# LuoGroup2023/PanTax

Hardware: AMD Instinct MI355X
Metric: PAO wall-time (s) + Mreads/s: packed reads + DB (graphs and their unique-trio index) resident in HBM -> abundance tables; the metric's own GAF -> abundance quantity is value_gaf_to_tables (files -> tables, never `value`) (higher is better)
Workload: dtype int64+f64

## Files before the change

### pantax_amd/csrc/common.hpp

```cpp
#pragma once
#include <hip/hip_runtime.h>
#include <cstdint>
#include <cstdio>
#include <map>
#include <functional>
#include <mutex>
#include <cstring>
#include <atomic>
#include <string>
#include <vector>
#include "../../include/pantax_hip.h"

#ifndef TRIO_LH_PACK
#define TRIO_LH_PACK 0
#endif
namespace ptx {

struct Ctx;
#if TRIO_LH_PACK
using trio_len_t = uint2;
#else
using trio_len_t = uint32_t;
#endif

// ... 36 lines not shown
    void release() {
        if (p && owned) dev_cache_free(p, cap, dev);
        p = nullptr;
        n = 0;
        cap = 0;
        owned = true;
    }
    void view(void *ptr, size_t count) {
        release();
        p = static_cast<T *>(ptr);
        n = count;
        owned = false;
    }
    hipError_t alloc(size_t count) {
        if (count <= n && p) return hipSuccess;
        release();
        hipError_t e = dev_cache_alloc((void **)&p, (count ? count : 1) * sizeof(T), &cap, &dev);
        if (e == hipSuccess) n = count ? count : 1;
        return e;
    }
    size_t bytes() const { return n * sizeof(T); }
    void take(DevBuf &o) { release(); p = o.p; n = o.n; cap = o.cap; dev = o.dev; owned = o.owned; o.p = nullptr; o.n = 0; o.cap = 0; o.owned = true; }
};

struct PinBuf {
    uint8_t *p = nullptr;
    size_t n = 0;
    PinBuf() = default;
    PinBuf(const PinBuf &) = delete;
    PinBuf &operator=(const PinBuf &) = delete;
    ~PinBuf() { release(); }
    void release() { if (p) (void)hipHostFree(p); p = nullptr; n = 0; }
    hipError_t reserve(size_t bytes) {
        if (bytes <= n && p) return hipSuccess;
        release();
        size_t want = bytes < 65536 ? 65536 : bytes;
        hipError_t e = hipHostMalloc((void **)&p, want, hipHostMallocDefault);
        if (e == hipSuccess) n = want;
        return e;
    }
};

struct TimedLaunch {
    const char *name;
    hipEvent_t start, stop;
};

struct CtxConfig {
    bool trace = false;
    int stage_threads = 32;
    int stage_ch_mb = 0;
    bool stream_prio = true;
    int dev_cache_gb = -1;
    bool numa_bind = true;
    uint64_t gaf_piece_bytes = 0;
    int db_groups = 0;
    uint64_t db_path_steps_max = 0;
    std::string trio_path;
    std::string trio_rows;
    int uniq_hash = -1;
    std::string mask;
    std::string row_sort;
    std::string objective;
    std::string read_strain_route, evidence_route, depth_route, near_miss_route, hap_pairs_route, fit_route, bootstrap_route, dropout_route;
    uint64_t bootstrap_rows_max = 0;
    uint64_t dropout_patterns_max = 0;
    bool dropout_yardstick = false;
    int hap_pairs_chunk = 0;
    int depth_grid = 0;
    int near_miss_words = 0;
    bool cov_general = false;
    std::string cov_long;
    int covl_shape = -1;
    bool cov_count = false;
    int cov_clean_async = -1;
    bool cov_self_clean = false;
    bool walk_sum_in_bin = false;
    int ncs_prefix_min = 48;
    bool ncs_no_prefix = false;
    bool cov_arena_verify = false;
    int cov_item_groups = 0;
    int tv_u = 4, tv_rounds = 4, tf_u = 8, tf_rounds = 1, rows_u = 1, tb_slots = 256, trio_xcd = 3, cov_shape = -1, covf_shape = -1, cov_xcd = 0, group_bucket_bits = 0;
    uint32_t tv_ablate = 0, cov_ablate = 0, ssn_ablate = 0;
    bool trio_two_pass = false;
    std::string bin_route;
    std::string node_pass;
    std::string node_bits;
    int node_bits_words = 0;
    std::string lad_shape;
    std::string scan_tile;
    std::string ssn_keys;
    bool ssn_poison_keys = false;
    int ssn_ties_async = -1;
    bool no_absent_skip = false;
    bool ssn_debug = false, scan_no_huge = false, flag_rank_chained = false, ratio_kernel = false, mask_pass = false, trio_free_at_filter = false,
         trio_after_step = false;
};
int ctx_set_option(CtxConfig &cfg, const char *name, const char *value);

struct NumaInfo {
    int node = -1;
    std::vector<int> cpus;
};

struct Ctx {
    std::recursive_mutex mu;
    CtxConfig cfg;
    NumaInfo numa;
    int device = 0;
    hipStream_t stream = nullptr;
    hipStream_t stream_main = nullptr;
    hipStream_t stream2 = nullptr;
    hipStream_t stream_up = nullptr;
    hipEvent_t ev_fork = nullptr;
    hipEvent_t ev_ssn_fork = nullptr, ev_ssn_join = nullptr;
    hipEvent_t ev_seq = nullptr;
    std::string err;
    std::mutex err_mu;
    bool timing = false;
    std::string timing_filter;
    std::vector<TimedLaunch> pending;
    std::vector<std::pair<hipEvent_t, hipEvent_t>> free_events;
    std::map<std::string, std::pair<uint64_t, double>> acc;
    int n_cu = 256;
    DevBuf<uint64_t> d_scalars;
    DevBuf<uint32_t> d_scan_ws;
    uint32_t scan_epoch = 0;
    DevBuf<uint32_t> d_scan_ws2;
    uint32_t scan_epoch2 = 0;
    PinBuf pin_down;
    PinBuf pin_text;
    PinBuf pin_up;
    size_t pin_up_off = 0;
    hipEvent_t pin_up_ev[2][2] = {{nullptr, nullptr}, {nullptr, nullptr}};
    bool pin_up_ev_set[2] = {false, false};
};

struct KTimer {
    Ctx *ctx;
    hipEvent_t start = nullptr, stop = nullptr;
    const char *name;
    KTimer(Ctx *c, const char *nm);
    ~KTimer();
};

int collect_timings(Ctx *ctx);

constexpr uint32_t BIN_PREFIX = 2048;
size_t bin_counter_words(uint32_t S);
size_t bin_result_words(uint32_t S);
struct Db; struct Reads;
int species_profile_launch(Ctx *ctx, const Db *db, const Reads *rd, const unsigned long long *d_counters, const double *d_avg_len, int filtered,
                           uint8_t *d_keep, double *d_absolute);
void species_profile_host(uint32_t S, const uint32_t *head_qlen, size_t n_head, const int64_t *read_count, const int64_t *base_sum,
                          const int64_t *less_multi, const int64_t *uniq_count, const double *avg_len, int filtered, uint8_t *keep_out,
                          double *absolute_out, double *abundance_out);
constexpr int PATH_TILE = 1024;
constexpr int LAD_MAXP = 64;
constexpr int LAD_WIDE_NW = 4;
constexpr int LAD_WIDEP = 64 * LAD_WIDE_NW;

struct LadBatch {
    uint32_t S = 0;
    bool prezeroed = false;
    std::vector<int32_t> h_p;
    std::vector<uint32_t> h_cand;
// ... 383 lines not shown
```

### pantax_amd/csrc/ctx.cpp

```cpp
#include <exception>
#include <cstdarg>
#include <algorithm>
#include <atomic>
#include <cstring>
#include <functional>
#include <chrono>
#include <condition_variable>
#include <cstdio>
#include <mutex>
#include <thread>
#include <unistd.h>
#include <fcntl.h>
#include <sched.h>
#include <pthread.h>
#include <sys/syscall.h>
#include <fstream>
#include <cctype>
#include <cstddef>
#include <cstdlib>
#include "common.hpp"
#include "lad.hpp"

namespace ptx {

static thread_local std::string g_init_err;
static thread_local std::string g_thread_err;
static thread_local const Ctx *g_thread_err_ctx = nullptr;

int fail(Ctx *ctx, int code, const char *fmt, ...) {
    char buf[1024];
    va_list ap;
    va_start(ap, fmt);
    vsnprintf(buf, sizeof(buf), fmt, ap);
    va_end(ap);
    if (ctx) {
        { std::lock_guard<std::mutex> g(ctx->err_mu); ctx->err = buf; }
        g_thread_err = buf; g_thread_err_ctx = ctx;
    } else g_init_err = buf;
    return code;
}

KTimer::KTimer(Ctx *c, const char *nm) : ctx(c), name(nm) {
    if (!ctx->timing) return;
    if (!ctx->timing_filter.empty()) {
        const std::string &f = ctx->timing_filter;
        const size_t len = std::strlen(nm);
        bool hit = false;
        for (size_t pos = 0; pos <= f.size() && !hit;) {
            const size_t bar = std::min(f.find('|', pos), f.size());
            hit = bar - pos == len && f.compare(pos, len, nm) == 0;
            pos = bar + 1;
        }
        if (!hit) return;
    }
    if (!ctx->free_events.empty()) {
        start = ctx->free_events.back().first;
        stop = ctx->free_events.back().second;
        ctx->free_events.pop_back();
    } else {
        if (hipEventCreate(&start) != hipSuccess || hipEventCreate(&stop) != hipSuccess) { start = stop = nullptr; return; }
    }
    (void)hipEventRecord(start, ctx->stream);
}
KTimer::~KTimer() {
    if (!start) return;
    (void)hipEventRecord(stop, ctx->stream);
    ctx->pending.push_back({name, start, stop});
}

int collect_timings(Ctx *ctx) {
    if (ctx->pending.empty()) return 0;
    PTX_HIP(ctx, hipStreamSynchronize(ctx->stream));
    for (auto &t : ctx->pending) {
        float ms = 0.f;
        if (hipEventElapsedTime(&ms, t.start, t.stop) == hipSuccess) {
            auto &a = ctx->acc[t.name];
            a.first += 1;
            a.second += ms;
        }
        ctx->free_events.push_back({t.start, t.stop});
    }
    ctx->pending.clear();
    return 0;
}

namespace {
enum OptKind { O_BOOL, O_INT, O_U32, O_U64, O_STR };
struct OptDesc { const char *name; OptKind kind; size_t off; };
#define OPT(nm, kind, field) {nm, kind, offsetof(CtxConfig, field)}
const OptDesc OPTIONS[] = {
    OPT("hip_trace", O_BOOL, trace), OPT("stage_threads", O_INT, stage_threads), OPT("stage_ch_mb", O_INT, stage_ch_mb), OPT("stream_prio", O_BOOL, stream_prio), OPT("numa_bind", O_BOOL, numa_bind), OPT("dev_cache_gb", O_INT, dev_cache_gb),
    OPT("gaf_piece_bytes", O_U64, gaf_piece_bytes), OPT("db_path_steps_max", O_U64, db_path_steps_max), OPT("db_groups", O_INT, db_groups), OPT("trio_path", O_STR, trio_path), OPT("trio_rows", O_STR, trio_rows), OPT("trio_two_pass", O_BOOL, trio_two_pass), OPT("uniq_hash", O_INT, uniq_hash),
    OPT("mask", O_STR, mask), OPT("row_sort", O_STR, row_sort), OPT("objective", O_STR, objective), OPT("read_strain_route", O_STR, read_strain_route), OPT("evidence_route", O_STR, evidence_route), OPT("depth_route", O_STR, depth_route), OPT("depth_grid", O_INT, depth_grid), OPT("near_miss_route", O_STR, near_miss_route), OPT("near_miss_words", O_INT, near_miss_words), OPT("hap_pairs_route", O_STR, hap_pairs_route), OPT("fit_route", O_STR, fit_route), OPT("bootstrap_route", O_STR, bootstrap_route), OPT("bootstrap_rows_max", O_U64, bootstrap_rows_max), OPT("dropout_route", O_STR, dropout_route), OPT("dropout_patterns_max", O_U64, dropout_patterns_max), OPT("dropout_yardstick", O_BOOL, dropout_yardstick), OPT("hap_pairs_chunk", O_INT, hap_pairs_chunk),
    OPT("cov_general", O_BOOL, cov_general), OPT("cov_long", O_STR, cov_long), OPT("covl_shape", O_INT, covl_shape), OPT("cov_count", O_BOOL, cov_count), OPT("cov_self_clean", O_BOOL, cov_self_clean), OPT("cov_clean_async", O_INT, cov_clean_async), OPT("cov_arena_verify", O_BOOL, cov_arena_verify), OPT("ncs_no_prefix", O_BOOL, ncs_no_prefix), OPT("ncs_prefix_min", O_INT, ncs_prefix_min), OPT("walk_sum_in_bin", O_BOOL, walk_sum_in_bin), OPT("cov_item_groups", O_INT, cov_item_groups), OPT("tv_u", O_INT, tv_u), OPT("tv_rounds", O_INT, tv_rounds), OPT("tf_u", O_INT, tf_u), OPT("tf_rounds", O_INT, tf_rounds),
    OPT("rows_u", O_INT, rows_u), OPT("tb_slots", O_INT, tb_slots), OPT("trio_xcd", O_INT, trio_xcd), OPT("cov_shape", O_INT, cov_shape),
    OPT("covf_shape", O_INT, covf_shape), OPT("cov_xcd", O_INT, cov_xcd), OPT("group_bucket_bits", O_INT, group_bucket_bits), OPT("tv_ablate", O_U32, tv_ablate),
    OPT("cov_ablate", O_U32, cov_ablate), OPT("ssn_ablate", O_U32, ssn_ablate), OPT("no_absent_skip", O_BOOL, no_absent_skip), OPT("node_pass", O_STR, node_pass), OPT("bin_route", O_STR, bin_route), OPT("node_bits", O_STR, node_bits), OPT("node_bits_words", O_INT, node_bits_words), OPT("lad_shape", O_STR, lad_shape), OPT("ssn_debug", O_BOOL, ssn_debug),
    OPT("ssn_keys", O_STR, ssn_keys), OPT("ssn_poison_keys", O_BOOL, ssn_poison_keys), OPT("ssn_ties_async", O_INT, ssn_ties_async),
    OPT("scan_no_huge", O_BOOL, scan_no_huge), OPT("scan_tile", O_STR, scan_tile), OPT("flag_rank_chained", O_BOOL, flag_rank_chained), OPT("ratio_kernel", O_BOOL, ratio_kernel),
    OPT("mask_pass", O_BOOL, mask_pass), OPT("trio_free_at_filter", O_BOOL, trio_free_at_filter), OPT("trio_after_step", O_BOOL, trio_after_step),
};
#undef OPT
}

int ctx_set_option(CtxConfig &cfg, const char *name, const char *value) {
    if (!name) return PANTAX_HIP_E_INVALID;
    static const CtxConfig defaults;
    for (const OptDesc &o : OPTIONS) {
        if (std::strcmp(o.name, name) != 0) continue;
        char *dst = reinterpret_cast<char *>(&cfg) + o.off;
        const char *def = reinterpret_cast<const char *>(&defaults) + o.off;
        char *end = nullptr;
        switch (o.kind) {
        case O_BOOL: *reinterpret_cast<bool *>(dst) = value ? !(value[0] == '0' || value[0] == '\0' || value[0] == 'n' || value[0] == 'f') : *reinterpret_cast<const bool *>(def); return 0;
        case O_INT: { if (!value) { *reinterpret_cast<int *>(dst) = *reinterpret_cast<const int *>(def); return 0; }
                      const long v = std::strtol(value, &end, 10); if (end == value) return PANTAX_HIP_E_INVALID; *reinterpret_cast<int *>(dst) = (int)v; return 0; }
        case O_U32: { if (!value) { *reinterpret_cast<uint32_t *>(dst) = *reinterpret_cast<const uint32_t *>(def); return 0; }
                      const unsigned long long v = std::strtoull(value, &end, 10); if (end == value) return PANTAX_HIP_E_INVALID; *reinterpret_cast<uint32_t *>(dst) = (uint32_t)v; return 0; }
        case O_U64: { if (!value) { *reinterpret_cast<uint64_t *>(dst) = *reinterpret_cast<const uint64_t *>(def); return 0; }
                      const unsigned long long v = std::strtoull(value, &end, 10); if (end == value) return PANTAX_HIP_E_INVALID; *reinterpret_cast<uint64_t *>(dst) = (uint64_t)v; return 0; }
        case O_STR: *reinterpret_cast<std::string *>(dst) = value ? value : ""; return 0;
        }
    }
    return PANTAX_HIP_E_INVALID;
}

static void config_from_env(CtxConfig &cfg) {
    for (const OptDesc &o : OPTIONS) {
        std::string env = "PANTAX_";
        for (const char *p = o.name; *p; ++p) env += (char)std::toupper((unsigned char)*p);
        if (const char *v = std::getenv(env.c_str())) (void)ctx_set_option(cfg, o.name, v);
    }
}

}

using namespace ptx;

extern "C" {

const char *pantax_hip_version(void) { return "pantax-hip 0.1.0 (gfx950)"; }

int pantax_hip_set_option(pantax_hip_ctx *ctx, const char *name, const char *value) {
    if (!ctx || !name) return PANTAX_HIP_E_INVALID;
    std::lock_guard<std::recursive_mutex> ptx_lock__(ctx->mu);
    const int rc = ctx_set_option(ctx->cfg, name, value);
    if (rc == 0 && std::strcmp(name, "dev_cache_gb") == 0) dev_cache_set_max(ctx->cfg.dev_cache_gb < 0 ? -1 : (long long)ctx->cfg.dev_cache_gb << 30);
    return rc == 0 ? 0 : fail(ctx, rc, "set_option: unknown option or unparsable value: %s=%s", name, value ? value : "(default)");
}

const char *pantax_hip_lad_shape_name(const pantax_hip_ctx *ctx, uint32_t n_species, int max_columns) {
    if (!ctx) return nullptr;
    return lad_shape_name(lad_shape(ctx->cfg.lad_shape, n_species, ctx->n_cu, max_columns));
}

const char *pantax_hip_last_error(const pantax_hip_ctx *ctx) {
    if (!ctx) return g_init_err.c_str();
    if (g_thread_err_ctx == ctx) return g_thread_err.c_str();
    std::lock_guard<std::mutex> g(const_cast<pantax_hip_ctx *>(ctx)->err_mu);
    g_thread_err = ctx->err;
    return g_thread_err.c_str();
}

int pantax_hip_init(pantax_hip_ctx **out, const int *device_ids, int n_devices) {
    if (!out) return PANTAX_HIP_E_INVALID;
    *out = nullptr;
    if (n_devices != 1) return fail(nullptr, PANTAX_HIP_E_INVALID, "one ctx drives one GPU (one process per GPU); n_devices=%d", n_devices);
    int count = 0;
    hipError_t e = hipGetDeviceCount(&count);
    if (e != hipSuccess || count == 0)
        return fail(nullptr, PANTAX_HIP_E_NO_DEVICE, "no HIP device visible (%s); this library has no CPU path",
                    e == hipSuccess ? "count=0" : hipGetErrorString(e));
    int dev = device_ids ? device_ids[0] : 0;
    if (dev < 0 || dev >= count) return fail(nullptr, PANTAX_HIP_E_INVALID, "device id %d out of range (count %d)", dev, count);
    hipDeviceProp_t prop;
    if ((e = hipGetDeviceProperties(&prop, dev)) != hipSuccess) return fail(nullptr, PANTAX_HIP_E_HIP, "hipGetDeviceProperties: %s", hipGetErrorString(e));
    if (strncmp(prop.gcnArchName, "gfx950", 6) != 0)
        return fail(nullptr, PANTAX_HIP_E_NO_DEVICE, "device %d is %s; this build carries gfx950 code only", dev, prop.gcnArchName);
    if ((e = hipSetDevice(dev)) != hipSuccess) return fail(nullptr, PANTAX_HIP_E_HIP, "hipSetDevice: %s", hipGetErrorString(e));
// ... 542 lines not shown
```

### pantax_amd/csrc/stage_cov.hip

```cpp
#include <chrono>
#include <cstdio>
#include <cstdlib>
#include "common.hpp"
#include "primitives.hpp"
#include "wave.hpp"
#include "cov_plan.hpp"
#include "cov_device.hpp"
#pragma clang diagnostic ignored "-Wbitwise-instead-of-logical"

namespace ptx {

template <bool WITH_TRIO, int U, int PASSES, int WIN, bool LONG = false>
__global__ void __launch_bounds__(COV_BLOCK) coverage_fast_kernel(
    const uint2 *__restrict__ items, const uint32_t *__restrict__ group_slot, const uint4 *__restrict__ read_rec, const uint2 *__restrict__ slot_rec,
    const uint32_t *__restrict__ node_id, const uint8_t *__restrict__ step_code, const uint8_t *__restrict__ active,
    const uint4 *__restrict__ node_rec, const uint64_t *__restrict__ bit_off, uint64_t V, unsigned long long *__restrict__ bases,
    uint32_t *__restrict__ bitmap, uint32_t *__restrict__ full, const uint2 *__restrict__ trio_ent, unsigned long long *__restrict__ trio_bases,
    unsigned long long *__restrict__ n_abort, uint32_t ablate, int blk_shift,
    const uint32_t *__restrict__ long_sum = nullptr, const uint32_t *__restrict__ long_len0 = nullptr, uint32_t only_long = 0u,
    uint32_t chunk_groups = 0u, uint32_t total_groups = 0u, uint32_t win_back = 0u, const uint32_t *__restrict__ item_sel = nullptr) {
    constexpr int WAVES = COV_BLOCK / 64;
    const int lane = threadIdx.x & 63, wave = threadIdx.x >> 6;
    uint32_t g0, n_groups;
    if constexpr (LONG) { g0 = blockIdx.x * chunk_groups; n_groups = min(g0 + chunk_groups, total_groups); }
    else { const uint2 item = items[item_sel ? item_sel[blockIdx.x] : blockIdx.x]; g0 = item.x; n_groups = item.y; }
    for (int i = threadIdx.x; i < (int)(cov_lds_bytes(WIN) / 4); i += COV_BLOCK) s_cov[i] = 0;
    uint32_t wlo = 0, win_n = 0, mark_n = 0, bit0_lo = 0, bwn = 0;
    uint64_t bw0 = 0;
#pragma unroll 1
    for (uint32_t g = g0; g < n_groups && win_n == 0; ++g) {
        const uint32_t gs = group_slot[g];
        if (gs == NO_SLOT) continue;
        const uint2 sr0 = slot_rec[gs];
        if ((int)sr0.x < 0 || !active[sr0.x]) continue;
        const uint32_t id0 = node_id[(uint64_t)g * 64], v0 = id0 + sr0.y, in_blk = id0 & ((1u << blk_shift) - 1u);
        const uint32_t back = LONG ? win_back : in_blk + 64u;
        wlo = (v0 > back ? v0 - back : 0u) & ~63u;
        win_n = WIN;
        const uint64_t b_lo = bit_off[wlo], b_hi = bit_off[min((uint64_t)wlo + WIN, V)];
        bw0 = b_lo >> 5;
        bit0_lo = (uint32_t)(bw0 << 5);
        bwn = COV_BWIN;
        mark_n = (b_hi - (bw0 << 5) <= (uint64_t)COV_BWIN * 32) ? (uint32_t)min((uint64_t)WIN, V - wlo) : 0u;
    }
    __builtin_amdgcn_fence(__ATOMIC_RELEASE, "workgroup", "local");
    __builtin_amdgcn_s_barrier();
    __builtin_amdgcn_fence(__ATOMIC_ACQUIRE, "workgroup", "local");
#ifndef COV_NO_PREFETCH
    uint32_t n_code[U], n_id[U], n_gs[U];
    {
        const uint32_t gw0 = g0 + (uint32_t)(wave * U);
#pragma unroll
        for (int u = 0; u < U; ++u) {
            const uint32_t g = gw0 + (uint32_t)u < n_groups ? gw0 + (uint32_t)u : (gw0 < n_groups ? gw0 : g0);
            const uint64_t t = (uint64_t)g * 64 + lane;
            n_code[u] = step_code[t]; n_id[u] = node_id[t]; n_gs[u] = group_slot[g];
        }
    }
#endif
#if !defined(COV_NO_PF2) && !defined(COV_NO_PREFETCH)
    constexpr bool PF2 = !LONG;
#else
    constexpr bool PF2 = false;
#endif
    uint32_t c_code[U], c_id[U], c_gs[U];
    uint4 c_rr[U];
    uint2 c_sr[U];
    bool c_run[U];
#pragma unroll
    for (int u = 0; u < U; ++u) c_run[u] = false;
    if constexpr (PF2) {
        const uint32_t gw0 = g0 + (uint32_t)(wave * U), gw1 = gw0 + (uint32_t)(WAVES * U);
#pragma unroll
        for (int u = 0; u < U; ++u) {
            c_code[u] = n_code[u]; c_id[u] = n_id[u]; c_gs[u] = n_gs[u];
            const uint32_t g = gw1 + (uint32_t)u < n_groups ? gw1 + (uint32_t)u : (gw0 < n_groups ? gw0 : g0);
            const uint64_t t = (uint64_t)g * 64 + lane;
            n_code[u] = step_code[t]; n_id[u] = node_id[t]; n_gs[u] = group_slot[g];
            const bool pad0 = c_code[u] == STEP_PAD;
            const bool run0 = (gw0 + (uint32_t)u < n_groups) & any1(!pad0) & none1(!pad0 & ((c_code[u] & STEP_LONG) != 0u));
            const uint32_t sl = slot_in_group(c_gs[u], c_code[u], lane);
            const uint32_t slot = (pad0 | !run0) ? (c_gs[u] == NO_SLOT ? 0u : c_gs[u]) : sl;
            c_rr[u] = read_rec[slot]; c_sr[u] = slot_rec[slot];
            c_run[u] = run0;
        }
    }
#pragma unroll 1
    for (int pass = 0;; ++pass) {
        const uint32_t gw = g0 + (uint32_t)((pass * WAVES + wave) * U);
        if (gw >= n_groups) break;
        uint32_t code[U], id[U], gs[U];
        bool run[U];
        uint4 rr[U];
        uint2 sr[U];
#ifndef COV_NO_PREFETCH
        if constexpr (PF2) {
            const uint32_t gn = gw + (uint32_t)(WAVES * U), g2 = gn + (uint32_t)(WAVES * U);
            uint32_t m_code[U], m_id[U], m_gs[U];
#pragma unroll
            for (int u = 0; u < U; ++u) {
                run[u] = c_run[u];
                code[u] = c_code[u]; id[u] = c_id[u]; gs[u] = c_gs[u]; rr[u] = c_rr[u]; sr[u] = c_sr[u];
                const uint32_t g = g2 + (uint32_t)u < n_groups ? g2 + (uint32_t)u : gw;
                const uint64_t t = (uint64_t)g * 64 + lane;
                m_code[u] = step_code[t]; m_id[u] = node_id[t]; m_gs[u] = group_slot[g];
                const bool padn = n_code[u] == STEP_PAD;
                const bool runn = (gn + (uint32_t)u < n_groups) & any1(!padn) & none1(!padn & ((n_code[u] & STEP_LONG) != 0u));
                const uint32_t sl = slot_in_group(n_gs[u], n_code[u], lane);
                const uint32_t slot = (padn | !runn) ? (n_gs[u] == NO_SLOT ? 0u : n_gs[u]) : sl;
                c_rr[u] = read_rec[slot]; c_sr[u] = slot_rec[slot];
                c_run[u] = runn;
                c_code[u] = n_code[u]; c_id[u] = n_id[u]; c_gs[u] = n_gs[u];
                n_code[u] = m_code[u]; n_id[u] = m_id[u]; n_gs[u] = m_gs[u];
            }
        } else
        {
            const uint32_t gn = gw + (uint32_t)(WAVES * U);
#pragma unroll
            for (int u = 0; u < U; ++u) {
                run[u] = gw + (uint32_t)u < n_groups;
                code[u] = n_code[u]; id[u] = n_id[u]; gs[u] = n_gs[u];
                const uint32_t g = gn + (uint32_t)u < n_groups ? gn + (uint32_t)u : gw;
                const uint64_t t = (uint64_t)g * 64 + lane;
                n_code[u] = step_code[t]; n_id[u] = node_id[t]; n_gs[u] = group_slot[g];
            }
        }
#else
#pragma unroll
        for (int u = 0; u < U; ++u) {
            const uint32_t g = gw + (uint32_t)u;
            run[u] = g < n_groups;
            const uint64_t t = (uint64_t)(run[u] ? g : gw) * 64 + lane;
            code[u] = step_code[t]; id[u] = node_id[t];
            gs[u] = group_slot[run[u] ? g : gw];
        }
#endif
        bool pad[U];
        uint32_t ll0[U], lsum[U];
#pragma unroll
        for (int u = 0; u < U; ++u) {
            pad[u] = code[u] == STEP_PAD;
            if constexpr (!PF2) {
                const bool has_long = any1(!pad[u] & ((code[u] & STEP_LONG) != 0u));
                run[u] = run[u] & any1(!pad[u]) & (LONG ? (has_long | (only_long == 0u)) : !has_long);
            }
            const uint32_t sl = slot_in_group(gs[u], code[u], lane);
            const uint32_t slot = (pad[u] | !run[u]) ? (gs[u] == NO_SLOT ? 0u : gs[u]) : sl;
            if constexpr (!PF2) { rr[u] = read_rec[slot]; sr[u] = slot_rec[slot]; }
            if constexpr (LONG) { ll0[u] = long_len0[slot]; lsum[u] = long_sum[slot]; }
        }
        uint32_t h_id1[U], h_id2[U], h_codes[U];
        if constexpr (LONG) {
#pragma unroll
            for (int u = 0; u < U; ++u) {
                const uint32_t gu = (uint32_t)__builtin_amdgcn_readfirstlane((int)(gw + (uint32_t)u));
                const uint64_t t0 = (uint64_t)(run[u] && gu != 0u ? gu : 1u) * 64;
                h_id1[u] = node_id[t0 - 1]; h_id2[u] = node_id[t0 - 2];
                h_codes[u] = *reinterpret_cast<const uint32_t *>(step_code + t0 - 4);
            }
        }
        uint4 nr[U];
        uint32_t v[U], act[U];
        bool ok[U];
#pragma unroll
        for (int u = 0; u < U; ++u) {
            ok[u] = run[u] & !pad[u] & ((int)sr[u].x >= 0);
            v[u] = ok[u] ? id[u] + sr[u].y : wlo;
            nr[u] = node_rec[v[u]];
            act[u] = active[ok[u] ? sr[u].x : 0u];
        }
        uint32_t idf[U], i0_[U], hv1[U], hv2[U];
        uint4 nrh1[U], nrh2[U];
        if constexpr (LONG) {
#pragma unroll
            for (int u = 0; u < U; ++u) {
                idf[u] = node_id[rr[u].x];
                const uint32_t gbase = (gw + (uint32_t)u) * 64u;
                const bool ok0 = __builtin_amdgcn_readfirstlane((int)ok[u]) != 0;
                i0_[u] = ok0 ? (uint32_t)__builtin_amdgcn_readfirstlane((int)(gbase - rr[u].x)) : 0u;
                const uint32_t delta0 = (uint32_t)__builtin_amdgcn_readfirstlane((int)sr[u].y);
                hv1[u] = i0_[u] >= 1u ? h_id1[u] + delta0 : wlo;
                hv2[u] = i0_[u] >= 2u ? h_id2[u] + delta0 : wlo;
                nrh1[u] = node_rec[hv1[u]]; nrh2[u] = node_rec[hv2[u]];
            }
        }
        uint32_t i_[U], nl[U], len0[U], nh[U], hx[U], tlo[U], thi[U];
        uint2 e0[U], e1[U];
        bool live[U], single[U], dead_read[U], cross[U];
        int dist[U];
#pragma unroll
        for (int u = 0; u < U; ++u) {
            const uint32_t gbase = (gw + (uint32_t)u) * 64u;
            i_[u] = gbase + (uint32_t)lane - rr[u].x;
            ok[u] = ok[u] & (act[u] != 0u);
            nl[u] = ok[u] ? nr[u].z : 0u;
            if constexpr (LONG) {
                dist[u] = (int)min(ok[u] ? i_[u] : 0u, (uint32_t)lane);
                cross[u] = ok[u] & (i_[u] > (uint32_t)lane);
                const uint32_t in_wave = __shfl(nl[u], lane - dist[u]);
                len0[u] = cross[u] ? ll0[u] : in_wave;
            } else
            len0[u] = __shfl(nl[u], lane - (int)i_[u]);
            uint32_t v2 = wave_shr1(wave_shr1(v[u]));
            uint32_t hw1 = wave_shr1(nr[u].w), hy1 = wave_shr1(nr[u].y);
            if constexpr (LONG) {
                v2 = lane == 0 ? hv2[u] : lane == 1 ? hv1[u] : v2;
                hw1 = lane == 0 ? nrh1[u].w : hw1; hy1 = lane == 0 ? nrh1[u].y : hy1;
            }
            single[u] = rr[u].y == 1u;
            dead_read[u] = !single[u] & (rr[u].z > len0[u]);
            live[u] = ok[u] & !dead_read[u] & !(single[u] & (rr[u].w < rr[u].z));
            nh[u] = 0; hx[u] = 0; tlo[u] = 0; thi[u] = 0;
            e0[u] = make_uint2(0u, 0u); e1[u] = e0[u];
            if (WITH_TRIO && !ABL(4u)) {
                hx[u] = hw1;
                tlo[u] = min(v[u], v2); thi[u] = max(v[u], v2);
                nh[u] = (live[u] & (i_[u] >= 2u) & ((nr_filter(hy1) & nr_pair_bit(tlo[u], thi[u])) != 0u)) ? nr_rows(hy1) : 0u;
                const EntPair ep = *reinterpret_cast<const EntPair *>(trio_ent + (nh[u] ? hx[u] : 0u));
                e0[u] = make_uint2(ep.a, ep.b); e1[u] = make_uint2(ep.c, ep.d);
            }
        }
#pragma unroll
        for (int u = 0; u < U; ++u) {
            const uint32_t k = rr[u].y, ps = rr[u].z, pe = rr[u].w, i = i_[u];
            if (any1(ok[u] & dead_read[u] & (i == 0u))) { if (ok[u] & dead_read[u] & (i == 0u)) atomicAdd(n_abort, 1ull); }
            const uint32_t contrib = (live[u] & !single[u]) ? (i == 0u ? nl[u] - ps : nl[u]) : 0u;
            const uint32_t pexcl = wave_incl_scan_dpp(contrib) - contrib;
            uint32_t seen = pexcl - __shfl(pexcl, lane - (LONG ? dist[u] : (int)i));
            if constexpr (LONG) seen = cross[u] ? lsum[u] - ps : seen;
            const uint32_t tgt = pe - ps;
            uint32_t aln = nl[u];
            if (i + 1u == k) aln = ((pe >= ps) & (tgt > seen)) ? tgt - seen : 0u;
            if (i == 0u) aln = single[u] ? tgt : nl[u] - ps;
            const uint32_t sidx = i == 0u ? ps : 0u;
            uint32_t hi = sidx + aln;
            if (hi > nl[u]) hi = nl[u];
            const bool markable = live[u] & (hi > sidx) & !(single[u] & !((ps < pe) & (pe <= nl[u])));
            const uint32_t dupd = code[u] & STEP_DIST;
            bool earlier = dupd != 0u, at_step0 = dupd == i;
            if constexpr (LONG) {
                const bool lc = (code[u] & STEP_LONG) != 0u;
                const uint32_t id_first = cross[u] ? idf[u] : __shfl(id[u], lane - dist[u]);
                earlier = lc ? (code[u] & 1u) != 0u : earlier;
                at_step0 = lc ? id[u] == id_first : at_step0;
            }
            const uint32_t rl = !live[u] ? 0u : !earlier ? aln : (at_step0 ? len0[u] - ps : nl[u]);
            const uint32_t off = v[u] - wlo;
            const bool inw = off < win_n;
            if (live[u] & !earlier & (aln != 0u) && !ABL(2u)) {
                if (inw & (aln < (1u << 18))) atomicAdd(&S_WIN(off), aln);
                else atomicAdd(&bases[v[u]], (unsigned long long)aln);
            }
// ... 228 lines not shown
    db->cov_arena_clean = false;
    db->cov_arena_sig = sig;
    if (rd->R && rd->T_pad && rd->n_long && rd->long_sums_db != 0 && rd->long_sums_db == db->uid) {
    } else if (rd->R && rd->T_pad && rd->n_long) {
        PTX_HIP(ctx, hipMemsetAsync(rd->d_long_sum.p, 0, rd->R * sizeof(uint32_t), ctx->stream));
        KTimer t(ctx, "walk_sum_kernel");
        const bool eager = (uint64_t)rd->n_long * 2 > rd->n_slots;
        hipLaunchKernelGGL((eager ? walk_sum_kernel<4, true> : walk_sum_kernel<4, false>), dim3(grid_for(rd->T_pad / 4 + 1, 256, ctx->n_cu * 16)), dim3(256), 0, ctx->stream, rd->T_pad, rd->d_g_group_slot.p,
                           rd->d_g_step_dup.p, rd->d_g_read_rec.p, rd->d_g_slot_rec.p, rd->d_g_node_id.p, db->d_node_len.p, rd->d_long_sum.p,
                           rd->d_long_len0.p);
    }
    PTX_HIP(ctx, hipGetLastError());
    db->cov_prepared = true;
    return 0;
}

int coverage_arena_clean_async(Ctx *ctx, Db *db) {
    if (!db->d_cov_arena.p || !db->cov_arena_total || !ctx->stream2) return 0;
    uint8_t *f_ptr = db->d_cov_arena.p;
    const size_t f_n = db->cov_arena_total;
    if (!db->ev_cov_read) PTX_HIP(ctx, hipEventCreateWithFlags(&db->ev_cov_read, hipEventDisableTiming));
    if (!db->ev_cov_clean) PTX_HIP(ctx, hipEventCreateWithFlags(&db->ev_cov_clean, hipEventDisableTiming));
    PTX_HIP(ctx, hipEventRecord(db->ev_cov_read, ctx->stream));
    PTX_HIP(ctx, hipStreamWaitEvent(ctx->stream2, db->ev_cov_read, 0));
    hipStream_t main_stream = ctx->stream;
    ctx->stream_main = main_stream; ctx->stream = ctx->stream2;
    int rc;
    rc = zero_fill(ctx, f_ptr, f_n);
    const hipError_t e = hipEventRecord(db->ev_cov_clean, ctx->stream2);
    ctx->stream = main_stream; ctx->stream_main = nullptr;
    if (rc != 0) return rc;
    PTX_HIP(ctx, e);
    db->cov_done = false;
    db->cov_arena_clean = true; db->cov_clean_pending = true;
    return 0;
}

struct CovLap {
    Ctx *ctx;
    bool on;
    std::chrono::steady_clock::time_point prev = std::chrono::steady_clock::now();
    void operator()(const char *what) {
        if (!on) return;
        (void)hipStreamSynchronize(ctx->stream);
        const auto now = std::chrono::steady_clock::now();
        std::fprintf(stderr, "[node_coverage]        %-28s %9.3f ms\n", what, std::chrono::duration<double, std::milli>(now - prev).count());
        prev = now;
    }
};

static int active_flags(Ctx *ctx, Db *db, const uint8_t *d_active, const uint8_t **out) {
    if (!d_active) {
        if (db->d_ones.n < db->S) { PTX_HIP(ctx, db->d_ones.alloc(db->S)); PTX_HIP(ctx, hipMemsetAsync(db->d_ones.p, 1, db->S, ctx->stream)); }
        d_active = db->d_ones.p;
    }
    *out = d_active;
    return 0;
}

struct ItemList { uint32_t n; const uint32_t *d; };
static int item_selection(Ctx *ctx, Db *db, const Reads *rd, ItemList *out) {
    *out = {rd->n_items, nullptr};
    if (db->item_sel_layout == rd->layout_id && rd->layout_id != 0) {
        *out = {db->item_sel_n, db->item_sel_on ? db->d_item_sel.p : nullptr};
    } else if (rd->h_item_block.size() == rd->n_items && rd->item_blk_shift > 0 && db->S && !db->h_range_start.empty()) {
        const CovItemSel s = cov_item_select(rd->h_item_block, rd->item_blk_shift, db->h_range_start, db->h_range_end);
        if (s.on && s.n_sel) PTX_TRY(upload(ctx, db->d_item_sel, s.sel.data(), s.sel.size()));
        *out = {s.n_sel, s.on && s.n_sel ? db->d_item_sel.p : nullptr};
        db->item_sel_layout = rd->layout_id; db->item_sel_n = s.n_sel; db->item_sel_on = s.on;
    }
    return 0;
}

struct CovFastTail {
    const uint2 *items; int blk_shift; const uint32_t *long_sum, *long_len0; uint32_t only_long, chunk_groups, total_groups, win_back; const uint32_t *item_sel;
};
template <int U, int PASSES, int WIN, bool LONG>
static void fast_launch_as(Ctx *ctx, Db *db, Reads *rd, const uint8_t *d_act, bool trio, int grid, const CovFastTail &t) {
    if (grid <= 0) return;
    const auto kernel = trio ? coverage_fast_kernel<true, U, PASSES, WIN, LONG> : coverage_fast_kernel<false, U, PASSES, WIN, LONG>;
    hipLaunchKernelGGL(kernel, dim3(grid), dim3(COV_BLOCK), cov_lds_bytes(WIN), ctx->stream, t.items, rd->d_g_group_slot.p, rd->d_g_read_rec.p,
                       rd->d_g_slot_rec.p, rd->d_g_node_id.p, rd->d_g_step_dup.p, d_act, db->d_node_rec.p, db->d_bit_off.p, db->V, db->d_bases.p,
                       db->d_bitmap.p, db->d_full.p, db->d_trio_ent.p, db->d_trio_bases.p, db->d_abort, ctx->cfg.cov_ablate ,
                       t.blk_shift, t.long_sum, t.long_len0, t.only_long, t.chunk_groups, t.total_groups, t.win_back, t.item_sel);
}

static int fast_launch(Ctx *ctx, Db *db, Reads *rd, const uint8_t *d_act, bool trio, const CovFastShape &f, const ItemList &list) {
    const CovFastTail t{rd->d_g_items.p, rd->item_blk_shift, nullptr, nullptr, 0u, 0u, 0u, 0u, list.d};
    const int grid = (int)list.n;
    const auto is = [&](int u, int passes, int win) { return f.u == u && f.passes == passes && f.win == win; };
    if (is(1, 8, 2048)) fast_launch_as<1, 8, 2048, false>(ctx, db, rd, d_act, trio, grid, t);
    else if (is(2, 4, 2048)) fast_launch_as<2, 4, 2048, false>(ctx, db, rd, d_act, trio, grid, t);
    else if (is(2, 8, 2048)) fast_launch_as<2, 8, 2048, false>(ctx, db, rd, d_act, trio, grid, t);
    else if (is(2, 8, 3072)) fast_launch_as<2, 8, 3072, false>(ctx, db, rd, d_act, trio, grid, t);
    else if (is(2, 8, 4096)) fast_launch_as<2, 8, 4096, false>(ctx, db, rd, d_act, trio, grid, t);
    else if (is(2, 4, 3072)) fast_launch_as<2, 4, 3072, false>(ctx, db, rd, d_act, trio, grid, t);
    else if (is(2, 8, 2304)) fast_launch_as<2, 8, 2304, false>(ctx, db, rd, d_act, trio, grid, t);
    else if (is(2, 8, 2560)) fast_launch_as<2, 8, 2560, false>(ctx, db, rd, d_act, trio, grid, t);
    else if (is(2, 4, 2304)) fast_launch_as<2, 4, 2304, false>(ctx, db, rd, d_act, trio, grid, t);
    else if (is(2, 4, 2560)) fast_launch_as<2, 4, 2560, false>(ctx, db, rd, d_act, trio, grid, t);
    else if (is(1, 8, 2304)) fast_launch_as<1, 8, 2304, false>(ctx, db, rd, d_act, trio, grid, t);
    else if (is(4, 4, 2304)) fast_launch_as<4, 4, 2304, false>(ctx, db, rd, d_act, trio, grid, t);
    else if (is(4, 4, 2048)) fast_launch_as<4, 4, 2048, false>(ctx, db, rd, d_act, trio, grid, t);
    else if (is(4, 4, 3072)) fast_launch_as<4, 4, 3072, false>(ctx, db, rd, d_act, trio, grid, t);
    else return fail(ctx, PANTAX_HIP_E_STATE, "coverage_launch: no short-read kernel of shape U = %d, PASSES = %d, WIN = %d", f.u, f.passes, f.win);
    return 0;
}

static int long_launch(Ctx *ctx, Db *db, Reads *rd, const uint8_t *d_act, bool trio, const CovPlan &plan) {
    if (!rd->d_long_sum.p) { PTX_HIP(ctx, rd->d_long_sum.alloc(rd->R)); PTX_HIP(ctx, rd->d_long_len0.alloc(rd->R)); }
    const CovLongShape &l = plan.lng;
    const uint32_t total_groups = (uint32_t)(rd->T_pad / 64);
    const int grid = (int)((total_groups + l.chunk_groups - 1) / l.chunk_groups);
    const CovFastTail t{nullptr, 0, rd->d_long_sum.p, rd->d_long_len0.p, plan.only_long ? 1u : 0u, l.chunk_groups, total_groups, l.win_back, nullptr};
    if (l.u == 1 && l.win == 2048) fast_launch_as<1, 1, 2048, true>(ctx, db, rd, d_act, trio, grid, t);
    else if (l.u == 1 && l.win == 3072) fast_launch_as<1, 1, 3072, true>(ctx, db, rd, d_act, trio, grid, t);
    else if (l.u == 1 && l.win == 4096) fast_launch_as<1, 1, 4096, true>(ctx, db, rd, d_act, trio, grid, t);
    else if (l.u == 2 && l.win == 2048) fast_launch_as<2, 1, 2048, true>(ctx, db, rd, d_act, trio, grid, t);
    else if (l.u == 2 && l.win == 4096) fast_launch_as<2, 1, 4096, true>(ctx, db, rd, d_act, trio, grid, t);
    else if (l.u == 2 && l.win == 3072) fast_launch_as<2, 1, 3072, true>(ctx, db, rd, d_act, trio, grid, t);
    else return fail(ctx, PANTAX_HIP_E_STATE, "coverage_launch: no long-walk kernel of shape U = %d, WIN = %d", l.u, l.win);
    return 0;
}

static int count_launch(Ctx *ctx, Db *db) {
    PTX_HIP(ctx, db->d_cov.alloc(db->V));
    KTimer t(ctx, "popcount_kernel");
    if (long_node_shape(db->L, db->V, ctx->cfg.ncs_prefix_min, ctx->cfg.ncs_no_prefix))
        hipLaunchKernelGGL(popcount_long_kernel, dim3(grid_for((db->V + 63) / 64, 4, ctx->n_cu * 8)), dim3(256), 0, ctx->stream, db->V,
                           db->d_bit_off.p, db->d_full.p, db->d_bitmap.p, db->d_cov.p);
    else
        hipLaunchKernelGGL(popcount_kernel, dim3(grid_for(db->V, 256, ctx->n_cu * 8)), dim3(256), 0, ctx->stream, db->V,
                           db->d_bit_off.p, db->d_full.p, db->d_bitmap.p, db->d_cov.p);
    return 0;
}

int coverage_launch(Ctx *ctx, Db *db, Reads *rd, const uint8_t *d_active, bool with_trio, bool defer_count) {
    if (!rd->grouped) return fail(ctx, PANTAX_HIP_E_STATE, "node_coverage: these reads are a slice kept as plain columns (to be routed to their owner), not resident reads");
    const bool trace = ctx->cfg.trace && !defer_count;
    CovLap lap{ctx, trace};
    if (!db->cov_prepared) PTX_TRY(coverage_prepare(ctx, db, rd, with_trio));
    lap("arena + zero fill");
    db->cov_prepared = false;
    db->cov_stage = false;
    db->trio_free_valid = false;
    const bool trio = with_trio && db->U;
    const uint8_t *d_act_fast = d_active;
    if (rd->R && rd->T_pad) PTX_TRY(active_flags(ctx, db, d_active, &d_act_fast));
    const CtxConfig &cfg = ctx->cfg;
    const CovPlan plan = cov_plan(rd->T_pad, rd->n_long, rd->n_slots, rd->n_items, rd->R, cfg.cov_general, cfg.cov_long, cfg.covf_shape, cfg.covl_shape,
                                  cfg.cov_shape, cfg.cov_xcd);
    if (plan.run_fast) {
        KTimer t(ctx, "coverage_fast_kernel");
        ItemList list;
        PTX_TRY(item_selection(ctx, db, rd, &list));
        if (trace) std::fprintf(stderr, "[node_coverage]        %u of %u items launched\n", list.n, rd->n_items);
        PTX_TRY(fast_launch(ctx, db, rd, d_act_fast, trio, plan.fast, list));
    }
    if (plan.run_long) {
        KTimer t(ctx, "coverage_long_kernel");
        PTX_TRY(long_launch(ctx, db, rd, d_act_fast, trio, plan));
    }
    if (plan.run_step) {
        KTimer t(ctx, "coverage_step_kernel");
        PTX_TRY(coverage_step_launch(ctx, db, rd, d_active, trio, plan));
    }
    PTX_HIP(ctx, hipGetLastError());
// ... 11 lines not shown
```

Before: 6830.

## Speculatively prefetch node records using first-slot delta in coverage kernel

Adds a third prefetch stage (PF3) to the coverage fast kernel. It guesses each group's vertex from the block's first active slot delta and prefetches node_rec one pipeline stage early, falling back to the exact slot_rec/active lookups only when a wave sees a different slot. It also sets a waves-per-EU attribute for small-U kernels and makes the wave index uniform via readfirstlane. The aim is to hide the dependent node_rec load latency, at the cost of extra registers, a redundant load whenever the speculation misses, and a new cov_spec=miss option that forces the fallback path.

Result: faster. 6912 (median of 6 runs) (+1.2%).

```diff
diff --git a/pantax_amd/csrc/common.hpp b/pantax_amd/csrc/common.hpp
--- a/pantax_amd/csrc/common.hpp
+++ b/pantax_amd/csrc/common.hpp
@@ -142,6 +142,7 @@
     int cov_item_groups = 0;
     int tv_u = 4, tv_rounds = 4, tf_u = 8, tf_rounds = 1, rows_u = 1, tb_slots = 256, trio_xcd = 3, cov_shape = -1, covf_shape = -1, cov_xcd = 0, group_bucket_bits = 0;
     uint32_t tv_ablate = 0, cov_ablate = 0, ssn_ablate = 0;
+    std::string cov_spec;
     bool trio_two_pass = false;
     std::string bin_route;
     std::string node_pass;
diff --git a/pantax_amd/csrc/ctx.cpp b/pantax_amd/csrc/ctx.cpp
--- a/pantax_amd/csrc/ctx.cpp
+++ b/pantax_amd/csrc/ctx.cpp
@@ -94,7 +94,7 @@
     OPT("mask", O_STR, mask), OPT("row_sort", O_STR, row_sort), OPT("objective", O_STR, objective), OPT("read_strain_route", O_STR, read_strain_route), OPT("evidence_route", O_STR, evidence_route), OPT("depth_route", O_STR, depth_route), OPT("depth_grid", O_INT, depth_grid), OPT("near_miss_route", O_STR, near_miss_route), OPT("near_miss_words", O_INT, near_miss_words), OPT("hap_pairs_route", O_STR, hap_pairs_route), OPT("fit_route", O_STR, fit_route), OPT("bootstrap_route", O_STR, bootstrap_route), OPT("bootstrap_rows_max", O_U64, bootstrap_rows_max), OPT("dropout_route", O_STR, dropout_route), OPT("dropout_patterns_max", O_U64, dropout_patterns_max), OPT("dropout_yardstick", O_BOOL, dropout_yardstick), OPT("hap_pairs_chunk", O_INT, hap_pairs_chunk),
     OPT("cov_general", O_BOOL, cov_general), OPT("cov_long", O_STR, cov_long), OPT("covl_shape", O_INT, covl_shape), OPT("cov_count", O_BOOL, cov_count), OPT("cov_self_clean", O_BOOL, cov_self_clean), OPT("cov_clean_async", O_INT, cov_clean_async), OPT("cov_arena_verify", O_BOOL, cov_arena_verify), OPT("ncs_no_prefix", O_BOOL, ncs_no_prefix), OPT("ncs_prefix_min", O_INT, ncs_prefix_min), OPT("walk_sum_in_bin", O_BOOL, walk_sum_in_bin), OPT("cov_item_groups", O_INT, cov_item_groups), OPT("tv_u", O_INT, tv_u), OPT("tv_rounds", O_INT, tv_rounds), OPT("tf_u", O_INT, tf_u), OPT("tf_rounds", O_INT, tf_rounds),
     OPT("rows_u", O_INT, rows_u), OPT("tb_slots", O_INT, tb_slots), OPT("trio_xcd", O_INT, trio_xcd), OPT("cov_shape", O_INT, cov_shape),
-    OPT("covf_shape", O_INT, covf_shape), OPT("cov_xcd", O_INT, cov_xcd), OPT("group_bucket_bits", O_INT, group_bucket_bits), OPT("tv_ablate", O_U32, tv_ablate),
+    OPT("covf_shape", O_INT, covf_shape), OPT("cov_spec", O_STR, cov_spec), OPT("cov_xcd", O_INT, cov_xcd), OPT("group_bucket_bits", O_INT, group_bucket_bits), OPT("tv_ablate", O_U32, tv_ablate),
     OPT("cov_ablate", O_U32, cov_ablate), OPT("ssn_ablate", O_U32, ssn_ablate), OPT("no_absent_skip", O_BOOL, no_absent_skip), OPT("node_pass", O_STR, node_pass), OPT("bin_route", O_STR, bin_route), OPT("node_bits", O_STR, node_bits), OPT("node_bits_words", O_INT, node_bits_words), OPT("lad_shape", O_STR, lad_shape), OPT("ssn_debug", O_BOOL, ssn_debug),
     OPT("ssn_keys", O_STR, ssn_keys), OPT("ssn_poison_keys", O_BOOL, ssn_poison_keys), OPT("ssn_ties_async", O_INT, ssn_ties_async),
     OPT("scan_no_huge", O_BOOL, scan_no_huge), OPT("scan_tile", O_STR, scan_tile), OPT("flag_rank_chained", O_BOOL, flag_rank_chained), OPT("ratio_kernel", O_BOOL, ratio_kernel),
diff --git a/pantax_amd/csrc/stage_cov.hip b/pantax_amd/csrc/stage_cov.hip
--- a/pantax_amd/csrc/stage_cov.hip
+++ b/pantax_amd/csrc/stage_cov.hip
@@ -11,6 +11,9 @@
 namespace ptx {
 
 template <bool WITH_TRIO, int U, int PASSES, int WIN, bool LONG = false>
+#if !defined(COV_NO_PF3) && !defined(COV_NO_PF2) && !defined(COV_NO_PREFETCH)
+__attribute__((amdgpu_waves_per_eu((U <= 2 && !LONG) ? 6 : 1)))
+#endif
 __global__ void __launch_bounds__(COV_BLOCK) coverage_fast_kernel(
     const uint2 *__restrict__ items, const uint32_t *__restrict__ group_slot, const uint4 *__restrict__ read_rec, const uint2 *__restrict__ slot_rec,
     const uint32_t *__restrict__ node_id, const uint8_t *__restrict__ step_code, const uint8_t *__restrict__ active,
@@ -18,21 +21,28 @@
     uint32_t *__restrict__ bitmap, uint32_t *__restrict__ full, const uint2 *__restrict__ trio_ent, unsigned long long *__restrict__ trio_bases,
     unsigned long long *__restrict__ n_abort, uint32_t ablate, int blk_shift,
     const uint32_t *__restrict__ long_sum = nullptr, const uint32_t *__restrict__ long_len0 = nullptr, uint32_t only_long = 0u,
-    uint32_t chunk_groups = 0u, uint32_t total_groups = 0u, uint32_t win_back = 0u, const uint32_t *__restrict__ item_sel = nullptr) {
+    uint32_t chunk_groups = 0u, uint32_t total_groups = 0u, uint32_t win_back = 0u, const uint32_t *__restrict__ item_sel = nullptr,
+    uint32_t spec_miss = 0u) {
     constexpr int WAVES = COV_BLOCK / 64;
+#if !defined(COV_NO_PF3) && !defined(COV_NO_PF2) && !defined(COV_NO_PREFETCH)
+    const int lane = threadIdx.x & 63, wave = LONG ? (int)(threadIdx.x >> 6) : __builtin_amdgcn_readfirstlane((int)(threadIdx.x >> 6));
+#else
     const int lane = threadIdx.x & 63, wave = threadIdx.x >> 6;
+#endif
     uint32_t g0, n_groups;
     if constexpr (LONG) { g0 = blockIdx.x * chunk_groups; n_groups = min(g0 + chunk_groups, total_groups); }
     else { const uint2 item = items[item_sel ? item_sel[blockIdx.x] : blockIdx.x]; g0 = item.x; n_groups = item.y; }
     for (int i = threadIdx.x; i < (int)(cov_lds_bytes(WIN) / 4); i += COV_BLOCK) s_cov[i] = 0;
     uint32_t wlo = 0, win_n = 0, mark_n = 0, bit0_lo = 0, bwn = 0;
     uint64_t bw0 = 0;
+    uint32_t s0 = 0xFFFFFFFFu, dlt0 = 0;
 #pragma unroll 1
     for (uint32_t g = g0; g < n_groups && win_n == 0; ++g) {
         const uint32_t gs = group_slot[g];
         if (gs == NO_SLOT) continue;
         const uint2 sr0 = slot_rec[gs];
         if ((int)sr0.x < 0 || !active[sr0.x]) continue;
+        s0 = sr0.x; dlt0 = sr0.y;
         const uint32_t id0 = node_id[(uint64_t)g * 64], v0 = id0 + sr0.y, in_blk = id0 & ((1u << blk_shift) - 1u);
         const uint32_t back = LONG ? win_back : in_blk + 64u;
         wlo = (v0 > back ? v0 - back : 0u) & ~63u;
@@ -43,6 +53,7 @@
         bwn = COV_BWIN;
         mark_n = (b_hi - (bw0 << 5) <= (uint64_t)COV_BWIN * 32) ? (uint32_t)min((uint64_t)WIN, V - wlo) : 0u;
     }
+    if (spec_miss) s0 = 0xFFFFFFFFu;
     __builtin_amdgcn_fence(__ATOMIC_RELEASE, "workgroup", "local");
     __builtin_amdgcn_s_barrier();
     __builtin_amdgcn_fence(__ATOMIC_ACQUIRE, "workgroup", "local");
@@ -63,9 +74,16 @@
 #else
     constexpr bool PF2 = false;
 #endif
+#if !defined(COV_NO_PF3)
+    constexpr bool PF3 = PF2;
+#else
+    constexpr bool PF3 = false;
+#endif
+    const auto guess_v = [&](uint32_t id) { const uint32_t vg = id + dlt0; return vg < V ? vg : wlo; };
     uint32_t c_code[U], c_id[U], c_gs[U];
     uint4 c_rr[U];
     uint2 c_sr[U];
+    uint4 c_nr[U];
     bool c_run[U];
 #pragma unroll
     for (int u = 0; u < U; ++u) c_run[u] = false;
@@ -81,9 +99,12 @@
             const bool run0 = (gw0 + (uint32_t)u < n_groups) & any1(!pad0) & none1(!pad0 & ((c_code[u] & STEP_LONG) != 0u));
             const uint32_t sl = slot_in_group(c_gs[u], c_code[u], lane);
             const uint32_t slot = (pad0 | !run0) ? (c_gs[u] == NO_SLOT ? 0u : c_gs[u]) : sl;
-            c_rr[u] = read_rec[slot]; c_sr[u] = slot_rec[slot];
+            c_rr[u] = read_rec[slot];
+            if constexpr (PF3) c_sr[u] = make_uint2(slot_rec[slot].x, 0u); else c_sr[u] = slot_rec[slot];
+            if constexpr (PF3) c_nr[u] = node_rec[guess_v(c_id[u])];
             c_run[u] = run0;
         }
+        if constexpr (PF3) __builtin_amdgcn_sched_barrier(0);
     }
 #pragma unroll 1
     for (int pass = 0;; ++pass) {
@@ -93,6 +114,7 @@
         bool run[U];
         uint4 rr[U];
         uint2 sr[U];
+        uint4 nrg[U];
 #ifndef COV_NO_PREFETCH
         if constexpr (PF2) {
             const uint32_t gn = gw + (uint32_t)(WAVES * U), g2 = gn + (uint32_t)(WAVES * U);
@@ -101,6 +123,7 @@
             for (int u = 0; u < U; ++u) {
                 run[u] = c_run[u];
                 code[u] = c_code[u]; id[u] = c_id[u]; gs[u] = c_gs[u]; rr[u] = c_rr[u]; sr[u] = c_sr[u];
+                if constexpr (PF3) nrg[u] = c_nr[u];
                 const uint32_t g = g2 + (uint32_t)u < n_groups ? g2 + (uint32_t)u : gw;
                 const uint64_t t = (uint64_t)g * 64 + lane;
                 m_code[u] = step_code[t]; m_id[u] = node_id[t]; m_gs[u] = group_slot[g];
@@ -108,11 +131,14 @@
                 const bool runn = (gn + (uint32_t)u < n_groups) & any1(!padn) & none1(!padn & ((n_code[u] & STEP_LONG) != 0u));
                 const uint32_t sl = slot_in_group(n_gs[u], n_code[u], lane);
                 const uint32_t slot = (padn | !runn) ? (n_gs[u] == NO_SLOT ? 0u : n_gs[u]) : sl;
-                c_rr[u] = read_rec[slot]; c_sr[u] = slot_rec[slot];
+                c_rr[u] = read_rec[slot];
+                if constexpr (PF3) c_sr[u] = make_uint2(slot_rec[slot].x, 0u); else c_sr[u] = slot_rec[slot];
+                if constexpr (PF3) c_nr[u] = node_rec[guess_v(n_id[u])];
                 c_run[u] = runn;
                 c_code[u] = n_code[u]; c_id[u] = n_id[u]; c_gs[u] = n_gs[u];
                 n_code[u] = m_code[u]; n_id[u] = m_id[u]; n_gs[u] = m_gs[u];
             }
+            if constexpr (PF3) __builtin_amdgcn_sched_barrier(0);
         } else
         {
             const uint32_t gn = gw + (uint32_t)(WAVES * U);
@@ -136,6 +162,7 @@
         }
 #endif
         bool pad[U];
+        uint32_t slot_[U];
         uint32_t ll0[U], lsum[U];
 #pragma unroll
         for (int u = 0; u < U; ++u) {
@@ -148,6 +175,7 @@
             const uint32_t slot = (pad[u] | !run[u]) ? (gs[u] == NO_SLOT ? 0u : gs[u]) : sl;
             if constexpr (!PF2) { rr[u] = read_rec[slot]; sr[u] = slot_rec[slot]; }
             if constexpr (LONG) { ll0[u] = long_len0[slot]; lsum[u] = long_sum[slot]; }
+            slot_[u] = slot;
         }
         uint32_t h_id1[U], h_id2[U], h_codes[U];
         if constexpr (LONG) {
@@ -165,9 +193,24 @@
 #pragma unroll
         for (int u = 0; u < U; ++u) {
             ok[u] = run[u] & !pad[u] & ((int)sr[u].x >= 0);
+            if constexpr (PF3) {
+                if (none1(ok[u] & (sr[u].x != s0))) {
+                    v[u] = ok[u] ? id[u] + dlt0 : wlo;
+                    nr[u] = nrg[u];
+                    asm volatile("" : "+v"(nr[u].x), "+v"(nr[u].y), "+v"(nr[u].z), "+v"(nr[u].w));
+                } else {
+                    v[u] = ok[u] ? id[u] + slot_rec[slot_[u]].y : wlo;
+                    nr[u] = node_rec[v[u]];
+                    const uint32_t a = active[ok[u] ? sr[u].x : 0u];
+                    asm volatile("" : "+v"(nr[u].x), "+v"(nr[u].y), "+v"(nr[u].z), "+v"(nr[u].w));
+                    ok[u] = ok[u] & (a != 0u);
+                }
+                act[u] = 1u;
+            } else {
             v[u] = ok[u] ? id[u] + sr[u].y : wlo;
             nr[u] = node_rec[v[u]];
             act[u] = active[ok[u] ? sr[u].x : 0u];
+            }
         }
         uint32_t idf[U], i0_[U], hv1[U], hv2[U];
         uint4 nrh1[U], nrh2[U];
@@ -562,7 +605,8 @@
     hipLaunchKernelGGL(kernel, dim3(grid), dim3(COV_BLOCK), cov_lds_bytes(WIN), ctx->stream, t.items, rd->d_g_group_slot.p, rd->d_g_read_rec.p,
                        rd->d_g_slot_rec.p, rd->d_g_node_id.p, rd->d_g_step_dup.p, d_act, db->d_node_rec.p, db->d_bit_off.p, db->V, db->d_bases.p,
                        db->d_bitmap.p, db->d_full.p, db->d_trio_ent.p, db->d_trio_bases.p, db->d_abort, ctx->cfg.cov_ablate ,
-                       t.blk_shift, t.long_sum, t.long_len0, t.only_long, t.chunk_groups, t.total_groups, t.win_back, t.item_sel);
+                       t.blk_shift, t.long_sum, t.long_len0, t.only_long, t.chunk_groups, t.total_groups, t.win_back, t.item_sel,
+                       ctx->cfg.cov_spec == "miss" ? 1u : 0u );
 }
 
 static int fast_launch(Ctx *ctx, Db *db, Reads *rd, const uint8_t *d_act, bool trio, const CovFastShape &f, const ItemList &list) {
```
